# linomp/INF560-approximate-pattern-matching

Measured on AMD Instinct MI355X. Metric: window-DP-cells/sec, higher is better.
Workload: dtype u32

## Files before the change

### inf560-approximate-pattern-matching_amd/csrc/apm_verify.hip

```cpp
#include <algorithm>
#include "apm_wave.h"
#include "apm_sieve.h"
#include "apm_launch.h"

#ifndef APM_WORK_CH
#define APM_WORK_CH 8u
#endif
#ifndef APM_WORK_CH8
#define APM_WORK_CH8 8u
#endif
#ifndef APM_VERIFY_PIPE
#define APM_VERIFY_PIPE 2
#endif
#ifndef APM_FUSED_PIPE
#define APM_FUSED_PIPE 1
#endif
#ifndef APM_VERIFY_AHEAD
#define APM_VERIFY_AHEAD 2
#endif
#ifndef APM_FUSED_S_WAVES
#define APM_FUSED_S_WAVES 6
#endif
#ifndef APM_DEDUP_PREFETCH
#define APM_DEDUP_PREFETCH(band, sampled, fused) (!(fused) && !(sampled))
#endif
#ifndef APM_DEDUP_WIDE
#define APM_DEDUP_WIDE(band, sampled, fused) ((band) >= 1)
#endif

struct ApmBufText {
    __amdgpu_buffer_rsrc_t rs;
    uint32_t off;
    static constexpr bool kBlocks = true;
    __device__ __forceinline__ bool can16(int) const { return true; }
    __device__ __forceinline__ void load16(uint32_t (&T)[4]) const { load16_at(0, T); }
    __device__ __forceinline__ void load16_at(int x0, uint32_t (&T)[4]) const {
        const uint32_t a0 = (off + (uint32_t)x0) & ~3u, sh = (off + (uint32_t)x0) & 3u;
        const u32x4 lo = __builtin_amdgcn_raw_buffer_load_b128(rs, (int)a0, 0, 0);
        const uint32_t hi = __builtin_amdgcn_raw_buffer_load_b32(rs, (int)(a0 + 16u), 0, 0);
        T[0] = __builtin_amdgcn_alignbyte(lo.y, lo.x, sh);
        T[1] = __builtin_amdgcn_alignbyte(lo.z, lo.y, sh);
        T[2] = __builtin_amdgcn_alignbyte(lo.w, lo.z, sh);
        T[3] = __builtin_amdgcn_alignbyte(hi, lo.w, sh);
    }
    __device__ __forceinline__ int byte(int x) const { return (int)__builtin_amdgcn_raw_buffer_load_b8(rs, (int)(off + (uint32_t)x), 0, 0); }
};

struct ApmWin { uint32_t w[6]; };

template <int BAND>
struct ApmVerifyCore {
    static constexpr int NSH = 2 * BAND + 1;
    static constexpr bool PAIRS = BAND >= 1;
    const ApmVerifyArgs &a;
    __amdgpu_buffer_rsrc_t rs;
    uint32_t avail;
    const uint32_t *s_kext;
    const uint4 *s_masks;
    const uint8_t *s_pat;
    uint32_t *s_cnt;
    int lane;
    const uint32_t *s_kinfo;
    const uint2 *s_pinfo;

    __device__ __forceinline__ void load_global(uint32_t a0, ApmWin &o) const {
        const u32x4 lo = __builtin_amdgcn_raw_buffer_load_b128(rs, (int)a0, 0, 0);
        const v2u32 hi = __builtin_amdgcn_raw_buffer_load_b64(rs, (int)(a0 + 16u), 0, 0);
        o.w[0] = lo.x; o.w[1] = lo.y; o.w[2] = lo.z; o.w[3] = lo.w; o.w[4] = hi.x; o.w[5] = hi.y;
    }
    __device__ __forceinline__ int gbyte(uint32_t pos) const {
        return (int)__builtin_amdgcn_raw_buffer_load_b8(rs, (int)pos, 0, 0);
    }

    template <typename LoadWin>
    __device__ __forceinline__ bool stage1(uint32_t kid, uint32_t s, const ApmWin &win, LoadWin &&load_win) const {
        typedef unsigned long long u64;
        const uint32_t kx = s_kext[kid];
        const int at = (int)(kx & 0xffffu), len = (int)((kx >> 16) & 0xffu), n = (int)((kx >> 24) & 31u), side = (int)(kx >> 29);
        if ((u64)s + (u64)len > (u64)avail) return false;
        const uint32_t sh = s & 3u;
        uint32_t A[4], B[4];
#pragma unroll
        for (int i = 0; i < 4; ++i) A[i] = __builtin_amdgcn_alignbyte(win.w[i + 1], win.w[i], sh);
        apm_lds_dwords<4>(s_pat, at, B);
        const uint4 mk = s_masks[len < 16 ? len : 16];
        if ((((A[0] ^ B[0]) & mk.x) | ((A[1] ^ B[1]) & mk.y) | ((A[2] ^ B[2]) & mk.z) | ((A[3] ^ B[3]) & mk.w)) != 0u) return false;
        for (int x = 16; x < len; ++x)
            if (gbyte(s + (uint32_t)x) != (int)s_pat[at + x]) return false;
        if (!PAIRS || side == 0) return true;
        if (n == 31) {
            const uint32_t kp = a.kpart[kid];
            const int poff = (int)(s_pinfo[s_kinfo[kid] & 0xfffu].x & 0xffffu), ap = (int)(kp & 0xffffu), nn = (int)(kp >> 16), ap1 = ap + nn;
            const bool fwd = side == 1;
            auto T = [&](int i) { return fwd ? gbyte(s + (uint32_t)len + (uint32_t)i) : gbyte(s - 1u - (uint32_t)i); };
            auto P = [&](int i) { return fwd ? (int)s_pat[poff + ap + i] : (int)s_pat[poff + ap1 - 1 - i]; };
            int i = 0;
            while (i < nn && T(i) == P(i)) ++i;
            if (i >= nn - 1) return true;
            bool ok = true;
            for (int j = i + 1; j < nn && ok; ++j) ok = T(j) == P(j);
            if (ok) return true;
            ok = true;
            for (int j = i + 1; j < nn && ok; ++j) ok = T(j - 1) == P(j);
            if (ok) return true;
            ok = true;
            for (int j = i; j < nn && ok; ++j) ok = T(j + 1) == P(j);
            return ok;
        }
        uint32_t P[4], T[5];
        ApmWin tw;
        if (side == 1) {
            const uint32_t tp = s + (uint32_t)len;
            if (len == 0 || APM_SKIP(a, 1024)) tw = win;
            else load_win(tp & ~3u, tw);
            apm_lds_dwords<4>(s_pat, at + len, P);
#pragma unroll
            for (int i = 0; i < 5; ++i) T[i] = __builtin_amdgcn_alignbyte(tw.w[i + 1], tw.w[i], tp & 3u);
        } else {
            uint32_t Q[4], Wd[5];
            apm_lds_dwords<4>(s_pat, at - 16, Q);
            if (s >= 20u) {
                const uint32_t tp = s - 20u;
                if (APM_SKIP(a, 1024)) tw = win;
                else load_win(tp & ~3u, tw);
#pragma unroll
                for (int i = 0; i < 5; ++i) Wd[i] = __builtin_amdgcn_alignbyte(tw.w[i + 1], tw.w[i], tp & 3u);
            } else {
#pragma unroll
                for (int i = 0; i < 5; ++i) Wd[i] = 0u;
                for (int i = 20 - (int)s; i < 20; ++i) {
                    const uint32_t b = (uint32_t)gbyte(s - 20u + (uint32_t)i);
#pragma unroll
                    for (int d = 0; d < 5; ++d)
                        if ((i >> 2) == d) Wd[d] |= b << (8 * (i & 3));
                }
            }
#pragma unroll
            for (int z = 0; z < 4; ++z) P[z] = apm_bswap(Q[3 - z]);
#pragma unroll
            for (int z = 0; z < 5; ++z) T[z] = apm_bswap(Wd[4 - z]);
        }
        if (n >= 4) {
            auto nz4 = [](uint32_t x) { return apm_udot4((((x & 0x7f7f7f7fu) + 0x7f7f7f7fu) | x) >> 7 & 0x01010101u, 0x08040201u); };
            const uint32_t z0 = nz4(P[0] ^ T[0]);
            if (z0 & (z0 - 1u)) {
                const uint32_t i = (uint32_t)__builtin_ctz(z0);
                const uint32_t z1 = nz4(P[0] ^ (T[0] << 8));
                const uint32_t z2 = nz4(P[0] ^ __builtin_amdgcn_alignbyte(T[1], T[0], 1u));
                if (((z1 >> (i + 1u)) != 0u) && ((z2 >> i) != 0u)) return false;
            }
        }
        return apm_ext1_core16(P, T, n);
    }


    __device__ __forceinline__ bool dp_match(uint32_t kid, uint32_t s, int dl, uint32_t &wpat, uint32_t &wj, uint32_t &word) const {
        const uint32_t ki = s_kinfo[kid];
        const int kpat = (int)(ki & 0xfffu), koff = (int)((ki >> 12) & 0x1ffu), kunit = (int)((ki >> 21) & 7u);
        const uint2 pinf = s_pinfo[kpat];
        const int poff = (int)(pinf.x & 0xffffu), m = (int)(pinf.x >> 16);
        const int64_t je_p = min(a.je, a.nrel - m + 1);
        const int64_t j = (int64_t)s - koff - dl;
        if (j < a.jb || j >= je_p) return false;
        wpat = (uint32_t)kpat;
        wj = (uint32_t)j;
        word = (uint32_t)(kunit * NSH + dl + BAND);
#ifdef APM_MEASURE
        if (APM_SKIP(a, 256)) atomicAdd(&a.stats[2], 1ull);
#endif
        return apm_banded_verify<BAND>(ApmBufText{rs, (uint32_t)j}, s_pat, poff, m, a.k);
    }

    template <bool PREF>
    __device__ __forceinline__ bool nominates(uint32_t bpat, uint32_t bj, int idx) const {
        const uint32_t kid = s_pinfo[bpat].y + (uint32_t)(idx / NSH);
        const int dd = idx % NSH - BAND;
        const int64_t o = (int64_t)bj + (int)((s_kinfo[kid] >> 12) & 0x1ffu) + dd;
        if (o < 0) return false;
        ApmWin w2;
        load_global((uint32_t)o & ~3u, w2);
        if constexpr (PAIRS && PREF) {
            const uint32_t kx = s_kext[kid];
            const uint32_t len = (kx >> 16) & 0xffu, side = kx >> 29;
            const bool ask = side != 0u && ((kx >> 24) & 31u) != 31u && (side == 1u ? len != 0u : o >= 20);
            const uint32_t pa = ask ? (side == 1u ? (uint32_t)o + len : (uint32_t)o - 20u) & ~3u : 0xffffff00u;
            ApmWin wp;
            load_global(pa, wp);
            return stage1(kid, (uint32_t)o, w2, [&](uint32_t a0, ApmWin &o2) {
                if (a0 == pa) o2 = wp;
                else load_global(a0, o2);
            });
        }
        return stage1(kid, (uint32_t)o, w2, [&](uint32_t a0, ApmWin &o2) { load_global(a0, o2); });
    }

    template <bool WIDE, bool PREF>
    __device__ __forceinline__ void count_matches(bool hit, uint32_t wpat, uint32_t wj, uint32_t word) const {
        for (unsigned long long m2 = __builtin_amdgcn_ballot_w64(hit); m2; m2 &= m2 - 1ull) {
            const int src = __builtin_ctzll(m2);
            const uint32_t bpat = (uint32_t)__builtin_amdgcn_readlane((int)wpat, src), bj = (uint32_t)__builtin_amdgcn_readlane((int)wj, src);
            const uint32_t bord = (uint32_t)__builtin_amdgcn_readlane((int)word, src);
            if (hit && wpat == bpat && wj == bj && word > bord) hit = false;
        }
        unsigned long long hm = __builtin_amdgcn_ballot_w64(hit);
        if constexpr (WIDE) {
            if (!hm) return;
#ifdef APM_MEASURE
            if (APM_SKIP(a, 32)) return;
#endif
            const unsigned long long pm = __builtin_amdgcn_ballot_w64(hit && word != 0u);
            unsigned long long dup = 0ull;
            uint32_t total = 0;
            for (unsigned long long mm = pm; mm; mm &= mm - 1ull) total += (uint32_t)__builtin_amdgcn_readlane((int)word, __builtin_ctzll(mm));
            for (uint32_t base = 0; base < total; base += 64u) {
                const uint32_t t = base + (uint32_t)lane;
                uint32_t msrc = 0, mfirst = 0, run = 0;
                for (unsigned long long mm = pm; mm; mm &= mm - 1ull) {
                    const int src = __builtin_ctzll(mm);
                    if (t >= run) { msrc = (uint32_t)src; mfirst = run; }
                    run += (uint32_t)__builtin_amdgcn_readlane((int)word, src);
                }
                const uint32_t bpat = (uint32_t)__builtin_amdgcn_ds_bpermute((int)(msrc << 2), (int)wpat);
                const uint32_t bj = (uint32_t)__builtin_amdgcn_ds_bpermute((int)(msrc << 2), (int)wj);
                const bool earlier = t < total && nominates<PREF>(bpat, bj, (int)(t - mfirst));
                unsigned long long em = __builtin_amdgcn_ballot_w64(earlier);
                while (em) {
                    const int l = __builtin_ctzll(em);
                    const uint32_t sl = (uint32_t)__builtin_amdgcn_readlane((int)msrc, l);
                    dup |= 1ull << sl;
                    em &= ~__builtin_amdgcn_ballot_w64(msrc == sl);
                }
            }
            const bool counts = hit && !((dup >> lane) & 1ull);
            if (counts) atomicAdd(&s_cnt[wpat], 1u);
#ifdef APM_REC
            apm_rec_push_wave(a.pos, counts, counts ? a.pats[wpat].index : 0u, (int64_t)wj);
#endif
#ifdef APM_MEASURE
            if (APM_SKIP(a, 256) && counts) atomicAdd(&a.stats[3], 1ull);
#endif
            return;
        }
        while (hm) {
            const int src = __builtin_ctzll(hm);
            hm &= hm - 1ull;
            const uint32_t bpat = (uint32_t)__builtin_amdgcn_readlane((int)wpat, src), bj = (uint32_t)__builtin_amdgcn_readlane((int)wj, src);
            const int n_before = __builtin_amdgcn_readlane((int)word, src);
#ifdef APM_MEASURE
            if (APM_SKIP(a, 32)) continue;
#endif
            const bool earlier = lane < n_before && nominates<false>(bpat, bj, lane);
            if (!__builtin_amdgcn_ballot_w64(earlier) && lane == 0) {
                atomicAdd(&s_cnt[bpat], 1u);
#ifdef APM_REC
                apm_rec_push(a.pos, a.pats[bpat].index, (int64_t)bj);
#endif
#ifdef APM_MEASURE
                if (APM_SKIP(a, 256)) atomicAdd(&a.stats[3], 1ull);
#endif
            }
        }
    }

};

__host__ __device__ constexpr int apm_verify_scap(int band) { return ((64 + 2 * band) / (2 * band + 1) + 63 + 7) & ~7; }

template <int BAND, int THREADS_T, bool SAMPLED, bool FUSED>
__device__ __forceinline__ void apm_verify_body(const ApmVerifyArgs &a, const ApmSieve2Args *sv, uint8_t *smem) {
    const int THREADS = THREADS_T ? THREADS_T : (int)blockDim.x;
    const int tid = threadIdx.x, lane = tid & 63;
    const int wv = __builtin_amdgcn_readfirstlane(tid >> 6);
    constexpr int NSH = 2 * BAND + 1;
    constexpr uint32_t FLUSH_AT = (64 + NSH - 1) / NSH;
    (void)FLUSH_AT;
    constexpr int SCAP = apm_verify_scap(BAND);
    uint8_t *s_img = smem + ((FUSED && !SAMPLED) ? 32768 : 0);
    const uint32_t *s_bmp = reinterpret_cast<const uint32_t *>(s_img);
    const uint16_t *s_prefix = reinterpret_cast<const uint16_t *>(s_img + a.o_prefix);
    const uint16_t *s_r2s = reinterpret_cast<const uint16_t *>(s_img + a.o_r2s);
    const uint16_t *s_slots = reinterpret_cast<const uint16_t *>(s_img + a.o_slots);
    const ApmKeyList keys{s_bmp, s_prefix, s_r2s, s_slots};
    const uint32_t *s_kext = reinterpret_cast<const uint32_t *>(s_img + a.o_kext);
    const uint8_t *s_pat = s_img + a.o_pat;
    const uint4 *s_masks = reinterpret_cast<const uint4 *>(s_img + a.o_masks);
    uint32_t *s_cnt = reinterpret_cast<uint32_t *>(s_img + a.image_len);
    uint2 *s_surv = reinterpret_cast<uint2 *>(s_cnt + ((a.n_pats + 3) & ~3)) + wv * SCAP;
    uint32_t *s_q = reinterpret_cast<uint32_t *>(reinterpret_cast<uint2 *>(s_cnt + ((a.n_pats + 3) & ~3)) + (THREADS / 64) * SCAP) + wv * 128;

    const uint32_t my_wave = blockIdx.x * (uint32_t)(THREADS / 64) + (uint32_t)wv;
    const uint32_t n_listed = (!FUSED && a.blist != nullptr) ? *a.blist_ctr : 0xffffffffu;
    bool cl_on = false;
    uint32_t cl_r = 0, cl_rstep = 0, cl_b = 0, cl_bstep = 1, cl_n = 0, cl_bs = 64;
    if constexpr (!FUSED && !SAMPLED) {
        if (a.clist) {
            const uint32_t R = (uint32_t)a.clist_regions, Wv = (uint32_t)gridDim.x * (uint32_t)(THREADS / 64);
            if (Wv >= R) {
                const uint32_t wpr = Wv / R;
                cl_on = my_wave < wpr * R;
                cl_r = my_wave % R;
                cl_rstep = R;
                cl_b = my_wave / R;
                cl_bstep = wpr;
            } else {
                cl_on = my_wave < R;
                cl_r = my_wave;
                cl_rstep = Wv;
            }
            if (cl_on) {
                cl_n = a.clist_cnt[cl_r];
                if (Wv >= R) {
                    const uint32_t per_wave = (cl_n + cl_bstep - 1u) / cl_bstep;
                    const uint32_t lo = (uint32_t)a.clist_min_batch;
                    cl_bs = per_wave >= 64u ? 64u : (per_wave < lo ? lo : per_wave);
                }
            }
        }
    }
    if constexpr (FUSED && !SAMPLED)
        apm_stage_image(reinterpret_cast<uint4 *>(smem), sv->bitmap, 2048, tid, THREADS);
    apm_stage_image(reinterpret_cast<uint4 *>(s_img), a.image, a.image_len >> 4, tid, THREADS);
    for (int i = tid; i < a.n_pats; i += THREADS) s_cnt[i] = 0u;
    __syncthreads();

    const __amdgpu_buffer_rsrc_t rs =
        __builtin_amdgcn_make_buffer_rsrc(const_cast<uint8_t *>(a.text), 0, (int)(uint32_t)a.avail_pad, 0x00020000);
    const uint32_t avail = (uint32_t)a.avail;
    const uint32_t cs = (uint32_t)a.code_shift;

    ApmVerifyCore<BAND> core{a, rs, avail, s_kext, s_masks, s_pat, s_cnt, lane, reinterpret_cast<const uint32_t *>(s_img + a.o_kinfo),
                             reinterpret_cast<const uint2 *>(s_img + a.o_pinfo)};
    typedef ApmWin Win;
    auto load_win = [&](uint32_t a0, Win &o) __attribute__((always_inline)) { core.load_global(a0, o); };

    uint32_t n_surv = 0;
    uint32_t item_lo = 0;
    constexpr uint32_t STEP = SAMPLED ? 8u : 2u;
    const bool listed = n_listed < (uint32_t)a.n_mask_blocks / 4u || (!FUSED && a.clist != nullptr);
    const uint32_t NB = FUSED ? (uint32_t)((sv->nchunks + 3) >> 2) : (listed ? n_listed : (uint32_t)a.n_mask_blocks);
    const uint32_t n_waves_launch = (uint32_t)(FUSED ? sv->n_main_blocks : (int)gridDim.x) * (uint32_t)(THREADS / 64);
    const uint32_t ch_fit = NB / (4u * n_waves_launch);
    const uint32_t CH = SAMPLED ? APM_WORK_CH8 : (listed ? 1u : (ch_fit >= APM_WORK_CH ? APM_WORK_CH : (ch_fit < 1u ? 1u : ch_fit)));
    const uint32_t NC = (NB + CH - 1u) / CH;
    const uint32_t NG = (uint32_t)a.work_groups, grp = (my_wave ^ (my_wave >> 5)) % NG;
    const uint32_t f_g = (uint32_t)(((uint64_t)NC * grp) / NG), n_g = (uint32_t)(((uint64_t)NC * (grp + 1u)) / NG) - f_g;
    uint32_t *const ctr = a.work + ((uint32_t)a.work_epoch & 1u) * (APM_WORK_GROUPS * APM_WORK_STRIDE) + grp * APM_WORK_STRIDE;
    if (blockIdx.x == 0 && tid < APM_WORK_GROUPS) a.work[(((uint32_t)a.work_epoch + 1u) & 1u) * (APM_WORK_GROUPS * APM_WORK_STRIDE) + (uint32_t)tid * APM_WORK_STRIDE] = 0u;
    auto grab = [&]() __attribute__((always_inline)) -> uint32_t {
        return lane == 0 ? __hip_atomic_fetch_add(ctr, 1u, __ATOMIC_RELAXED, __HIP_MEMORY_SCOPE_AGENT) : 0u;
    };
    uint32_t grab_v = grab();
    uint32_t it_b = 0, it_end = 0;
    bool it_done = false;
    constexpr bool STATIC_BLOCKS = FUSED && SAMPLED;
    const uint32_t n_waves_all = (uint32_t)(FUSED ? sv->n_main_blocks : (int)gridDim.x) * (uint32_t)(THREADS / 64);
    uint32_t st_b = my_wave;
    auto it_next = [&](uint32_t &b) __attribute__((always_inline)) -> bool {
        if constexpr (STATIC_BLOCKS) {
            if (st_b >= NB) return false;
            b = st_b;
            st_b += n_waves_all;
            return true;
        }
        if (it_b >= it_end) {
            if (it_done) return false;
            const uint32_t i = (uint32_t)__builtin_amdgcn_readfirstlane((int)grab_v);
            if (i >= n_g) { it_done = true; return false; }
            it_b = (f_g + i) * CH;
            it_end = it_b + CH < NB ? it_b + CH : NB;
            grab_v = grab();
        }
        b = it_b++;
        return true;
    };
    constexpr int AHEAD = FUSED ? 1 : (SAMPLED ? 4 : APM_VERIFY_AHEAD);
    constexpr uint32_t NONE = 0xffffffffu;
    uint32_t hm = 0, hm_q[AHEAD], hb_q[AHEAD];
    if constexpr (!FUSED) {
#pragma unroll
        for (int i = 0; i < AHEAD; ++i) {
            uint32_t b = NONE;
            hb_q[i] = it_next(b) ? (listed ? a.blist[b] : b) : NONE;
            hm_q[i] = hb_q[i] != NONE ? a.masks[(uint64_t)hb_q[i] * 64 + (uint64_t)lane] : 0u;
        }
    }
#ifdef APM_MEASURE
    if (APM_SKIP(a, 512) && lane == 0 && my_wave < APM_STATS_WAVES) a.stats[8 + 2 * my_wave] = wall_clock64();
#endif
    uint32_t blk = 0;
    uint32_t qcount = 0;
    const uint32_t nch32 = FUSED ? (uint32_t)sv->nchunks : 0u;
    const uint32_t tile0 = FUSED ? (uint32_t)sv->tile0 : 0u;
    constexpr bool PREF = FUSED && SAMPLED;
    u32x4 pf_r[4];
    uint32_t pf_sl[4];
    uint32_t pf_b = 0xffffffffu;
    bool pf_started = false;
    auto pf_issue = [&](uint32_t b) __attribute__((always_inline)) {
        const uint32_t g = tile0 + b * 4096u + 16u * (uint32_t)lane;
#pragma unroll
        for (int j = 0; j < 4; ++j) pf_r[j] = __builtin_amdgcn_raw_buffer_load_b128(rs, (int)(g + 1024u * j), 0, 0);
    };
    auto sieve_block = [&](uint32_t b0, uint32_t fb) __attribute__((always_inline)) -> uint32_t {
        const uint32_t g = b0 + 16u * (uint32_t)lane, c0 = fb * 4u;
        uint32_t out = 0;
        if constexpr (SAMPLED) {
            uint32_t sl[4];
#pragma unroll
            for (int j = 0; j < 4; ++j) sl[j] = pf_sl[j];
#pragma unroll
            for (int j = 0; j < 4; ++j) {
                const uint32_t slo = sl[j];
                const uint32_t w0 = s_bmp[slo & 2047u], w1 = s_bmp[(slo >> 16) & 2047u];
                const uint32_t h = ((w0 >> ((slo >> 11) & 31u)) & 1u) | (((w1 >> (slo >> 27)) & 1u) << 1);
                out |= (c0 + j < nch32 ? h : 0u) << (8 * j);
            }
            {
                uint32_t pend = out, cur = 0, curbit = 0, slo_c = 0, tsel = 0;
                bool act = false;
                for (;;) {
                    if (!act && pend) {
                        curbit = (uint32_t)__builtin_ctz(pend);
                        pend &= pend - 1u;
                        tsel = curbit & 1u;
                        const uint32_t j = curbit >> 3;
#pragma unroll
                        for (int q = 0; q < 4; ++q)
                            if (j == (uint32_t)q) slo_c = sl[q];
                        cur = keys.first(tsel ? (slo_c >> 16) : (slo_c & 0xffffu));
                        act = true;
                    }
                    if (!__builtin_amdgcn_ballot_w64(act)) break;
                    if (act && a.o_rc) {
                        const uint32_t kid = ApmKeyList::kid(cur, 11u), rr = ApmKeyList::r(cur, 11u);
                        const uint2 rc = reinterpret_cast<const uint2 *>(s_img + a.o_rc)[(kid * 8u + rr) * 2u + tsel];
                        if (((rc.x ^ slo_c) & rc.y) == 0u) act = false;
                        else if (ApmKeyList::last(cur)) { act = false; out &= ~(1u << curbit); }
                        else cur = keys.next(cur);
                    } else if (act) {
                        const uint32_t kid = ApmKeyList::kid(cur, 11u), rr = ApmKeyList::r(cur, 11u);
                        const uint32_t kx = s_kext[kid];
                        const int at = (int)(kx & 0xffffu), len = (int)((kx >> 16) & 0xffu);
                        const int sh8 = (int)(8u * tsel) - (int)rr;
                        uint32_t B[4];
                        apm_lds_dwords<4>(s_pat, at - sh8, B);
                        const uint32_t pc = apm_pack4(B[0], cs) | (apm_pack4(B[1], cs) << 8) | (apm_pack4(B[2], cs) << 16) | (apm_pack4(B[3], cs) << 24);
                        const int i0 = sh8 > 0 ? sh8 : 0, i1 = len + sh8 < 16 ? len + sh8 : 16;
                        const uint32_t mhi = i1 >= 16 ? 0xffffffffu : ((1u << (2 * i1)) - 1u), mlo = (1u << (2 * i0)) - 1u;
                        if ((((pc ^ slo_c) & mhi) & ~mlo) == 0u) act = false;
                        else if (ApmKeyList::last(cur)) { act = false; out &= ~(1u << curbit); }
                        else cur = keys.next(cur);
                    }
                }
            }
        } else {
            u32x4 r[4];
#pragma unroll
            for (int j = 0; j < 4; ++j) r[j] = __builtin_amdgcn_raw_buffer_load_b128(rs, (int)(g + 1024u * j), 0, 0);
            const v2u32 tl = __builtin_amdgcn_raw_buffer_load_b64(rs, (int)(b0 + 4096u), 0, 0);
            uint32_t slo[5];
#pragma unroll
            for (int j = 0; j < 4; ++j) slo[j] = apm_pack16(r[j].x, r[j].y, r[j].z, r[j].w, cs);
            slo[4] = apm_pack4(tl.x, cs) | (apm_pack4(tl.y, cs) << 8);
#pragma unroll
            for (int j = 0; j < 4; ++j) {
                const uint32_t hits = apm_lookup2_chunk(slo[j], (uint32_t)__builtin_amdgcn_readfirstlane((int)slo[j + 1]));
                out |= (c0 + j < nch32 ? hits >> 24 : 0u) << (8 * j);
                __builtin_amdgcn_sched_barrier(0);
            }
        }
        return out;
    };
    auto next_cand = [&](uint32_t &q, bool &hv) __attribute__((always_inline)) -> bool {
        if constexpr (!FUSED && !SAMPLED) {
            while (cl_on) {
                const uint32_t o = cl_b * cl_bs;
                if (o < cl_n) {
                    const uint32_t nb = cl_n - o < cl_bs ? cl_n - o : cl_bs;
                    hv = (uint32_t)lane < nb;
                    q = hv ? a.clist[(size_t)cl_r * a.clist_cap + o + (uint32_t)lane] : 0u;
                    cl_b += cl_bstep;
                    return true;
                }
                cl_r += cl_rstep;
                cl_b = 0;
                if (cl_r >= (uint32_t)a.clist_regions) { cl_on = false; break; }
                cl_n = a.clist_cnt[cl_r];
            }
        }
        while (qcount < 64u) {
            if (!__builtin_amdgcn_ballot_w64(hm != 0u)) {
                if constexpr (FUSED) {
                    uint32_t b;
                    if constexpr (PREF) {
                        if (!pf_started) {
                            pf_started = true;
                            uint32_t nb;
                            if (it_next(nb)) { pf_b = nb; pf_issue(nb); }
                        }
                        if (pf_b == 0xffffffffu) break;
                        b = pf_b;
#pragma unroll
                        for (int j = 0; j < 4; ++j) pf_sl[j] = apm_pack16(pf_r[j].x, pf_r[j].y, pf_r[j].z, pf_r[j].w, cs);
                        uint32_t nb;
                        if (it_next(nb)) { pf_b = nb; pf_issue(nb); }
                        else pf_b = 0xffffffffu;
                    } else if (!it_next(b)) break;
                    blk = tile0 + b * 4096u;
                    hm = sieve_block(blk, b);
                    continue;
                }
                if (hb_q[0] == NONE) break;
                blk = (uint32_t)(a.tile0 + (int64_t)hb_q[0] * 4096);
                hm = hm_q[0];
#pragma unroll
                for (int i = 0; i + 1 < AHEAD; ++i) { hm_q[i] = hm_q[i + 1]; hb_q[i] = hb_q[i + 1]; }
                {
                    uint32_t b = NONE;
                    hb_q[AHEAD - 1] = it_next(b) ? (listed ? a.blist[b] : b) : NONE;
                    hm_q[AHEAD - 1] = hb_q[AHEAD - 1] != NONE ? a.masks[(uint64_t)hb_q[AHEAD - 1] * 64 + (uint64_t)lane] : 0u;
                }
                continue;
            }
            const bool has = hm != 0u;
            const uint32_t t = has ? (uint32_t)__builtin_ctz(hm) : 0u;
            hm &= hm - 1u;
            apm_wave_append(s_q, qcount, has, (blk + (t >> 3) * 1024u + 16u * (uint32_t)lane + (SAMPLED ? (t & 1u) * 8u : (t & 7u) * 2u)) / STEP);
        }
        q = 0;
        hv = false;
        if (qcount == 0u) return false;
        const uint32_t nb = qcount < 64u ? qcount : 64u;
        hv = (uint32_t)lane < nb;
        if (hv) q = s_q[lane];
        if (qcount > 64u) {
            const uint32_t rest = s_q[64 + lane];
            if ((uint32_t)lane < qcount - 64u) s_q[lane] = rest;
        }
        qcount -= nb;
        return true;
    };
    bool done = false, active = false, have = false;
    uint32_t p = 0, str = 0, s = 0, pend = 0;
    uint32_t cur = 0;
    Win win, win_n, wk;
    constexpr uint32_t PSH = SAMPLED ? 3u : 1u;
    constexpr uint32_t KBITS = SAMPLED ? 11u : 15u;
    uint32_t q_n = 0;
    bool have_n = false;
    bool ex_n = true;
    constexpr int PIPE = FUSED ? APM_FUSED_PIPE : APM_VERIFY_PIPE;
    uint32_t q_nn = 0;
    bool have_nn = false, ex_nn = true;
    load_win(0u, win_n);
    for (;;) {
        if (n_surv * NSH - item_lo >= 64u || (done && n_surv)) {
            const uint32_t avail_items = n_surv * NSH - item_lo, proc = done ? avail_items : (avail_items & ~63u);
            for (uint32_t w0 = 0; w0 < proc; w0 += 64) {
                const uint32_t wi = item_lo + w0 + (uint32_t)lane;
                const bool live = w0 + (uint32_t)lane < proc;
                const uint2 e = live ? s_surv[wi / NSH] : make_uint2(0u, 0u);
                const int dl = (int)(wi % NSH) - BAND;
                uint32_t wpat = 0, wj = 0, word = 0;
                bool hit = live && core.dp_match(e.y, e.x, dl, wpat, wj, word);
#ifdef APM_MEASURE
                if (APM_SKIP(a, 64)) hit = false;
#endif
                core.template count_matches<APM_DEDUP_WIDE(BAND, SAMPLED, FUSED), APM_DEDUP_PREFETCH(BAND, SAMPLED, FUSED)>(hit, wpat, wj, word);
            }
            const uint32_t s_first = (item_lo + proc) / NSH, left = n_surv - s_first;
            const uint2 keep = (uint32_t)lane < left ? s_surv[s_first + (uint32_t)lane] : make_uint2(0u, 0u);
            if ((uint32_t)lane < left) s_surv[lane] = keep;
            item_lo = item_lo + proc - s_first * NSH;
            n_surv = left;
        }
        if (done) break;
        if (!active && pend) {
            const uint32_t par = (pend & 1u) ? 0u : 1u;
            pend &= pend - 1u;
            cur = keys.first((str >> (2u * par)) & 0xffffu);
            s = p + par;
            active = true;
            if constexpr (SAMPLED) {
                s = p - ApmKeyList::r(cur, KBITS);
                if (s > p) s = 0xffffffffu;
                load_win(s & ~3u, wk);
            }
        }
        if (!__builtin_amdgcn_ballot_w64(active)) {
            if (!ex_n) { done = true; continue; }
            p = q_n << PSH;
            have = have_n;
            win = win_n;
            if constexpr (PIPE == 2) {
                ex_n = ex_nn;
                q_n = q_nn;
                have_n = have_nn;
                load_win((q_n << PSH) & ~3u, win_n);
                ex_nn = next_cand(q_nn, have_nn);
            } else {
                ex_n = next_cand(q_n, have_n);
                load_win((q_n << PSH) & ~3u, win_n);
            }
            str = 0;
#pragma unroll
            for (int i = 0; i < 3; ++i) {
                const uint32_t b4 = __builtin_amdgcn_alignbyte(win.w[i + 1], win.w[i], p & 3u);
                str |= apm_pack4(b4, cs) << (8 * i);
            }
            const uint32_t x0 = str & 0xffffu, x1 = (str >> 2) & 0xffffu;
            pend = have ? (((s_bmp[x0 & 2047u] >> (x0 >> 11)) & 1u) | (SAMPLED ? 0u : (((s_bmp[x1 & 2047u] >> (x1 >> 11)) & 1u) << 1))) : 0u;
#ifdef APM_MEASURE
            if (APM_SKIP(a, 8)) pend = 0;
#endif
            continue;
        }
        bool ok = false;
        if (active) ok = core.stage1(ApmKeyList::kid(cur, KBITS), s, SAMPLED ? wk : win, load_win);
#ifdef APM_MEASURE
        if (APM_SKIP(a, 16)) ok = false;
#endif
        const unsigned long long mask = __builtin_amdgcn_ballot_w64(ok);
#ifdef APM_MEASURE
        if (APM_SKIP(a, 256) && mask && lane == 0) atomicAdd(&a.stats[1], (unsigned long long)__builtin_popcountll(mask));
#endif
        if (mask) {
            const uint32_t idx = n_surv + apm_wave_rank(mask);
            if (ok) s_surv[idx] = make_uint2(s, ApmKeyList::kid(cur, KBITS));
            n_surv += (uint32_t)__builtin_popcountll(mask);
        }
        if (active) {
            if (ApmKeyList::last(cur)) active = false;
            else {
                cur = keys.next(cur);
                if constexpr (SAMPLED) {
                    s = p - ApmKeyList::r(cur, KBITS);
                    if (s > p) s = 0xffffffffu;
                    load_win(s & ~3u, wk);
                }
            }
        }
    }

#ifdef APM_MEASURE
    if (APM_SKIP(a, 512) && lane == 0 && my_wave < APM_STATS_WAVES) a.stats[9 + 2 * my_wave] = wall_clock64();
#endif
    __syncthreads();
    for (int i = tid; i < a.n_pats; i += THREADS) {
        const uint32_t cnt = s_cnt[i];
        if (cnt) atomicAdd(&a.counts[a.pats[i].index], (unsigned long long)cnt);
    }
}

template <int BAND, int THREADS, bool SAMPLED>
__global__ __launch_bounds__(THREADS, (BAND == 1 && THREADS == 256 && !SAMPLED) ? 6 : 4) void apm_verify_kernel(ApmVerifyArgs a) {
    extern __shared__ __attribute__((aligned(16))) uint8_t smem[];
    apm_verify_body<BAND, THREADS, SAMPLED, false>(a, nullptr, smem);
}

static size_t apm_verify_lds_bytes_t(const ApmVerifyArgs &a, int threads) {
    return (size_t)a.image_len + (size_t)((a.n_pats + 3) & ~3) * 4 + (size_t)(threads / 64) * ((size_t)apm_verify_scap(a.band) * 8 + 128 * 4) +
           16;
}

template <typename Family>
static const void *apm_band_fn(int band, const Family &k) {
    switch (band) {
    case 0: return k.template fn<0>();
    case 1: return k.template fn<1>();
    case 2: return k.template fn<2>();
    case 3: return k.template fn<3>();
    default: return nullptr;
    }
}
struct ApmVerifyFamily {
    int threads, stride;
    template <int BAND>
    const void *fn() const {
        if (threads == 512) return stride == 8 ? (const void *)apm_verify_kernel<BAND, 512, true> : (const void *)apm_verify_kernel<BAND, 512, false>;
        return stride == 8 ? (const void *)apm_verify_kernel<BAND, 256, true> : (const void *)apm_verify_kernel<BAND, 256, false>;
    }
};
static const void *apm_verify_fn(int band, int threads, int stride) { return apm_band_fn(band, ApmVerifyFamily{threads, stride}); }

int apm_verify_geometry(const ApmVerifyArgs &a, int *threads) {
    const int blocks = apm_best_geometry([&](int t) { return apm_verify_fn(a.band, t, a.stride); }, 256, 512, 256,
                                         [&](int t) { return apm_verify_lds_bytes_t(a, t); }, 8, 0, threads);
    if (blocks) return blocks;
    *threads = 256;
    return 2;
}

hipError_t apm_launch_verify(const ApmVerifyArgs &a, int threads, int max_blocks, int *work_epoch, hipStream_t s) {
    if (a.n_pats <= 0) return hipSuccess;
    const void *fn = apm_verify_fn(a.band, threads, a.stride);
    if (!fn) return hipErrorInvalidValue;
    ApmVerifyArgs args = a;
    args.n_blocks = max_blocks < 1 ? 1 : max_blocks;
#ifdef APM_MEASURE
    if (const char *e = getenv("APM_VERIFY_GRID_PCT")) args.n_blocks = std::max(1, (int)((long)args.n_blocks * atoi(e) / 100));
    if (const char *e = getenv("APM_MEASURE_SKIP")) args.skip_mask = atoi(e);
#endif
    args.work_groups = std::min<long>(APM_WORK_GROUPS, (long)args.n_blocks * (threads / 64));
    args.work_epoch = *work_epoch;
    void *kargs[] = {&args};
    const hipError_t e = hipLaunchKernel(fn, dim3((unsigned)args.n_blocks), dim3((unsigned)threads), kargs, apm_verify_lds_bytes_t(a, threads), s);
    if (e == hipSuccess) ++*work_epoch;
    return e;
}

template <int BAND, bool SAMPLED>
__global__ __launch_bounds__(APM_FUSED_MAX_THREADS, SAMPLED ? (BAND == 0 ? 7 : (BAND == 1 ? APM_FUSED_S_WAVES : 5)) : (BAND == 0 ? 6 : 5)) void apm_fused_kernel(ApmFusedArgs f) {
    extern __shared__ __attribute__((aligned(16))) uint8_t smem[];
    if ((int)blockIdx.x >= f.s.n_main_blocks) {
        apm_tail_body(f.s.tail, (int)blockIdx.x - f.s.n_main_blocks, reinterpret_cast<uint4 *>(smem), (int)threadIdx.x);
        return;
    }
    apm_verify_body<BAND, 0, SAMPLED, true>(f.v, &f.s, smem);
}

struct ApmFusedFamily {
    int stride;
    template <int BAND>
    const void *fn() const { return stride == 8 ? (const void *)apm_fused_kernel<BAND, true> : (const void *)apm_fused_kernel<BAND, false>; }
};
static const void *apm_fused_fn(int band, int stride) { return apm_band_fn(band, ApmFusedFamily{stride}); }

size_t apm_fused_lds_bytes(const ApmFusedArgs &a, int threads) {
    const size_t need = (a.s.stride == 8 ? 0 : 32768) + apm_verify_lds_bytes_t(a.v, threads);
    return need < 4096 + 256 ? 4096 + 256 : need;
}

int apm_fused_geometry(const ApmFusedArgs &a, int *threads) {
    const void *fn = apm_fused_fn(a.v.band, a.s.stride);
    *threads = 0;
    if (!fn) return 0;
    apm_ensure_max_lds(fn);
#ifdef APM_MEASURE
    static const int forced = getenv("APM_FUSED_THREADS") ? atoi(getenv("APM_FUSED_THREADS")) : 0;
#else
    constexpr int forced = 0;
#endif
    return apm_best_geometry([&](int) { return fn; }, APM_FUSED_MAX_THREADS, 256, -64, [&](int t) { return apm_fused_lds_bytes(a, t); }, INT_MAX, forced, threads);
}

hipError_t apm_launch_fused(const ApmFusedArgs &a, int threads, int max_blocks, int *work_epoch, hipStream_t s) {
    if (a.s.nchunks <= 0 || a.v.n_pats <= 0) return hipSuccess;
    const void *fn = apm_fused_fn(a.v.band, a.s.stride);
    if (!fn || threads < 64 || threads > APM_FUSED_MAX_THREADS || (threads & 63)) return hipErrorInvalidValue;
    const size_t lds = apm_fused_lds_bytes(a, threads);
    const int64_t n_fb = (a.s.nchunks + 3) / 4, want = (n_fb + threads / 64 - 1) / (threads / 64);
    const int64_t nb = want < max_blocks ? want : (max_blocks < 1 ? 1 : max_blocks);
    ApmFusedArgs args = a;
    args.s.n_main_blocks = (int)nb;
    args.v.n_blocks = (int)nb;
#ifdef APM_MEASURE
    if (const char *e = getenv("APM_MEASURE_SKIP")) args.v.skip_mask = atoi(e);
#endif
    if (lds > 48 * 1024) apm_ensure_max_lds(fn);
    args.v.work_groups = (int)std::min<int64_t>(APM_WORK_GROUPS, nb * (threads / 64));
    args.v.work_epoch = *work_epoch;
    void *kargs[] = {&args};
    const hipError_t e = hipLaunchKernel(fn, dim3((unsigned)(nb + a.s.n_tail)), dim3((unsigned)threads), kargs, lds, s);
    if (e == hipSuccess) ++*work_epoch;
    return e;
}
```

Measured before the change: 704100000 billion.

## Deal candidate-list batches globally across waves using wave-wide prefix scans

Replaces the per-region static assignment of candidate-list batches to waves with a global dealing scheme. The total candidate count across all regions sets a single batch size. Each wave then takes batch indices wave, wave+W, and so on, finding the owning region through a wave-wide inclusive scan of per-region batch counts. This is meant to fix load imbalance when region counts are skewed or when there are fewer waves than regions. In exchange it adds a prologue that reads all region counts, plus extra scan and ballot work per batch.

```diff
diff --git a/inf560-approximate-pattern-matching_amd/csrc/apm_deal.h b/inf560-approximate-pattern-matching_amd/csrc/apm_deal.h
--- /dev/null
+++ b/inf560-approximate-pattern-matching_amd/csrc/apm_deal.h
@@ -0,0 +1,47 @@
+#ifndef APM_DEAL_H
+#define APM_DEAL_H
+
+#include <stdint.h>
+#include "apm_core.h"
+
+#define APM_DEAL_CHUNK 64u
+
+struct ApmDealBatch {
+    uint32_t region, off, len;
+};
+
+APM_HD uint32_t apm_deal_bs(uint32_t total, uint32_t waves, uint32_t min_batch) {
+    const uint32_t per = total / waves + (total % waves != 0u ? 1u : 0u);
+    return per >= 64u ? 64u : (per < min_batch ? min_batch : per);
+}
+
+APM_HD uint32_t apm_deal_batches(uint32_t cnt, uint32_t bs) { return (cnt + bs - 1u) / bs; }
+
+APM_HD uint32_t apm_deal_magic(uint32_t bs) { return 0xffffffffu / bs + 1u; }
+APM_HD uint32_t apm_deal_div(uint32_t n, uint32_t bs, uint32_t magic) { return bs == 1u ? n : (uint32_t)(((uint64_t)n * magic) >> 32); }
+APM_HD uint32_t apm_deal_batches_m(uint32_t cnt, uint32_t bs, uint32_t magic) { return apm_deal_div(cnt + bs - 1u, bs, magic); }
+
+APM_HD void apm_deal_cut(uint32_t cnt, uint32_t bs, uint32_t b, uint32_t &off, uint32_t &len) {
+    off = b * bs;
+    len = cnt - off < bs ? cnt - off : bs;
+}
+
+APM_HD bool apm_deal_batch(const uint32_t *cnt, uint32_t R, uint32_t waves, uint32_t min_batch, uint32_t wave, uint32_t i,
+                           uint32_t *bs, ApmDealBatch *out) {
+    uint64_t total = 0;
+    for (uint32_t r = 0; r < R; ++r) total += cnt[r];
+    *bs = apm_deal_bs(total > 0xffffffffull ? 0xffffffffu : (uint32_t)total, waves, min_batch);
+    uint64_t g = (uint64_t)wave + (uint64_t)i * waves;
+    for (uint32_t r = 0; r < R; ++r) {
+        const uint32_t nb = apm_deal_batches(cnt[r], *bs);
+        if (g < nb) {
+            out->region = r;
+            apm_deal_cut(cnt[r], *bs, (uint32_t)g, out->off, out->len);
+            return true;
+        }
+        g -= nb;
+    }
+    return false;
+}
+
+#endif
diff --git a/inf560-approximate-pattern-matching_amd/csrc/apm_verify.hip b/inf560-approximate-pattern-matching_amd/csrc/apm_verify.hip
--- a/inf560-approximate-pattern-matching_amd/csrc/apm_verify.hip
+++ b/inf560-approximate-pattern-matching_amd/csrc/apm_verify.hip
@@ -1,6 +1,7 @@
 #include <algorithm>
 #include "apm_wave.h"
 #include "apm_sieve.h"
+#include "apm_deal.h"
 #include "apm_launch.h"
 
 #ifndef APM_WORK_CH
@@ -290,37 +291,58 @@
 
     const uint32_t my_wave = blockIdx.x * (uint32_t)(THREADS / 64) + (uint32_t)wv;
     const uint32_t n_listed = (!FUSED && a.blist != nullptr) ? *a.blist_ctr : 0xffffffffu;
+    constexpr int CL_AHEAD = 8;
     bool cl_on = false;
-    uint32_t cl_r = 0, cl_rstep = 0, cl_b = 0, cl_bstep = 1, cl_n = 0, cl_bs = 64;
+    uint32_t cl_bs = 64, cl_magic = 0, cl_max = 0, cl_g = my_wave, cl_c0 = 0, cl_pre = 0, cl_r = 0, cl_o = 0, cl_len = 0;
+    const uint32_t cl_R = (!FUSED && !SAMPLED && a.clist) ? (uint32_t)a.clist_regions : 0u;
+    const uint32_t cl_W = (uint32_t)gridDim.x * (uint32_t)(THREADS / 64);
+    auto cl_count = [&](uint32_t c0) __attribute__((always_inline)) -> uint32_t {
+        return c0 + (uint32_t)lane < cl_R ? a.clist_cnt[c0 + (uint32_t)lane] : 0u;
+    };
+    auto cl_step = [&](uint32_t v) __attribute__((always_inline)) -> bool {
+        const uint32_t nb = apm_deal_batches_m(v, cl_bs, cl_magic), incl = apm_wave_incl_scan(nb);
+        const uint32_t tot = (uint32_t)__builtin_amdgcn_readlane((int)incl, 63), t = cl_g - cl_pre;
+        if (t >= tot) { cl_pre += tot; cl_c0 += APM_DEAL_CHUNK; return false; }
+        const int owner = __builtin_ctzll(__builtin_amdgcn_ballot_w64(t < incl));
+        cl_r = cl_c0 + (uint32_t)owner;
+        apm_deal_cut((uint32_t)__builtin_amdgcn_readlane((int)v, owner), cl_bs, t - (uint32_t)__builtin_amdgcn_readlane((int)(incl - nb), owner), cl_o, cl_len);
+        return true;
+    };
+    auto cl_find = [&]() __attribute__((always_inline)) -> bool {
+        while (cl_c0 < cl_R)
+            if (cl_step(cl_count(cl_c0))) return true;
+        return false;
+    };
+    uint32_t cl_v[CL_AHEAD] = {};
     if constexpr (!FUSED && !SAMPLED) {
-        if (a.clist) {
-            const uint32_t R = (uint32_t)a.clist_regions, Wv = (uint32_t)gridDim.x * (uint32_t)(THREADS / 64);
-            if (Wv >= R) {
-                const uint32_t wpr = Wv / R;
-                cl_on = my_wave < wpr * R;
-                cl_r = my_wave % R;
-                cl_rstep = R;
-                cl_b = my_wave / R;
-                cl_bstep = wpr;
-            } else {
-                cl_on = my_wave < R;
-                cl_r = my_wave;
-                cl_rstep = Wv;
-            }
-            if (cl_on) {
-                cl_n = a.clist_cnt[cl_r];
-                if (Wv >= R) {
-                    const uint32_t per_wave = (cl_n + cl_bstep - 1u) / cl_bstep;
-                    const uint32_t lo = (uint32_t)a.clist_min_batch;
-                    cl_bs = per_wave >= 64u ? 64u : (per_wave < lo ? lo : per_wave);
-                }
-            }
-        }
-    }
+        if (cl_R) {
+#pragma unroll
+            for (int j = 0; j < CL_AHEAD; ++j) cl_v[j] = cl_count(APM_DEAL_CHUNK * (uint32_t)j);
+        }
+    }
+    auto cl_start = [&]() __attribute__((always_inline)) {
+        if constexpr (!FUSED && !SAMPLED) {
+            if (!cl_R) return;
+            uint32_t sum = 0;
+#pragma unroll
+            for (int j = 0; j < CL_AHEAD; ++j) sum += cl_v[j];
+            for (uint32_t c0 = APM_DEAL_CHUNK * CL_AHEAD; c0 < cl_R; c0 += APM_DEAL_CHUNK) sum += cl_count(c0);
+            const uint32_t total = (uint32_t)__builtin_amdgcn_readlane((int)apm_wave_incl_scan(sum), 63);
+            cl_bs = apm_deal_bs(total, cl_W, (uint32_t)a.clist_min_batch);
+            cl_magic = apm_deal_magic(cl_bs);
+            cl_max = apm_deal_div(total, cl_bs, cl_magic) + cl_R;
+            if (cl_g >= cl_max) return;
+#pragma unroll
+            for (int j = 0; j < CL_AHEAD; ++j)
+                if (!cl_on && cl_c0 == APM_DEAL_CHUNK * (uint32_t)j && cl_c0 < cl_R) cl_on = cl_step(cl_v[j]);
+            if (!cl_on) cl_on = cl_find();
+        }
+    };
     if constexpr (FUSED && !SAMPLED)
         apm_stage_image(reinterpret_cast<uint4 *>(smem), sv->bitmap, 2048, tid, THREADS);
     apm_stage_image(reinterpret_cast<uint4 *>(s_img), a.image, a.image_len >> 4, tid, THREADS);
     for (int i = tid; i < a.n_pats; i += THREADS) s_cnt[i] = 0u;
+    cl_start();
     __syncthreads();
 
     const __amdgpu_buffer_rsrc_t rs =
@@ -473,19 +495,12 @@
     };
     auto next_cand = [&](uint32_t &q, bool &hv) __attribute__((always_inline)) -> bool {
         if constexpr (!FUSED && !SAMPLED) {
-            while (cl_on) {
-                const uint32_t o = cl_b * cl_bs;
-                if (o < cl_n) {
-                    const uint32_t nb = cl_n - o < cl_bs ? cl_n - o : cl_bs;
-                    hv = (uint32_t)lane < nb;
-                    q = hv ? a.clist[(size_t)cl_r * a.clist_cap + o + (uint32_t)lane] : 0u;
-                    cl_b += cl_bstep;
-                    return true;
-                }
-                cl_r += cl_rstep;
-                cl_b = 0;
-                if (cl_r >= (uint32_t)a.clist_regions) { cl_on = false; break; }
-                cl_n = a.clist_cnt[cl_r];
+            if (cl_on) {
+                hv = (uint32_t)lane < cl_len;
+                q = hv ? a.clist[(size_t)cl_r * a.clist_cap + cl_o + (uint32_t)lane] : 0u;
+                cl_g += cl_W;
+                cl_on = cl_g < cl_max && cl_find();
+                return true;
             }
         }
         while (qcount < 64u) {
```

Measured after the change: 712200000 billion, median of 6. 1.01x the previous value.
